# regras/NTT-based-polynomial-multiplier-FPGA

Hardware: AMD Instinct MI355X
Metric: polymults/sec (n=4096, 32-bit q) at 1/2/4/8 MI355X; % HBM roofline (higher is better)
Workload: dtype u32

## Files before the change

ntt-based-polynomial-multiplier-fpga_amd/csrc/arith_select.hpp:

```cpp
#pragma once
#include <stdint.h>

#ifndef NTTMUL_SPLIT16
#define NTTMUL_SPLIT16 4
#endif
#ifndef NTTMUL_C5_SQ
#define NTTMUL_C5_SQ 1
#endif

namespace nttmul {

constexpr int row_logs(int logn) {
  return logn <= 12 ? logn : (logn == 16 && NTTMUL_SPLIT16 == 5 ? 11 : 12);
}
constexpr int groups_g(int logs) { return (logs + 3) / 4; }
constexpr int groups_s(int logs, int g) {
  return logs / groups_g(logs) + (g < logs % groups_g(logs) ? 1 : 0);
}
constexpr bool p_signed_fw_entry(int logn, uint32_t idx) {
  if (idx < 2) return false;
  int st = 0;
  while ((2u << st) <= idx) st++;
  const int logs = row_logs(logn), local = st - (logn - logs);
  if (local < 0) return false;
  int g = 0, st0 = 0;
  while (st0 + groups_s(logs, g) <= local) st0 += groups_s(logs, g++);
  return local - st0 >= 1 && (idx & 1);
}

constexpr bool p3_fold_ok(uint64_t q) {
  if (q >= (1ull << 31) || q < 3) return false;
  const unsigned __int128 s1 = (unsigned __int128)4 * (q - 1) * (q - 1);
  const unsigned __int128 c32 = ((unsigned __int128)1 << 32) % q;
  const unsigned __int128 fold = (s1 >> 32) * c32 + 0xFFFFFFFFu;
  return fold + s1 < ((unsigned __int128)1 << 64);
}

enum class A32Kind { Plantard, Wide };

constexpr A32Kind a32_kind(uint64_t q) {
  return q >= (1ull << 31) ? A32Kind::Wide : A32Kind::Plantard;
}

}
```

ntt-based-polynomial-multiplier-fpga_amd/csrc/kernels.hip:

```cpp
#if defined(NTTMUL_HOOK_ROWS_LD) || defined(NTTMUL_HOOK_ROWS_ST) || defined(NTTMUL_HOOK_ROWS_INPUT) || \
    defined(NTTMUL_HOOK_ROWS_OUTPUT) || defined(NTTMUL_HOOK_XCHG) || defined(NTTMUL_HOOK_COLS_LD) || \
    defined(NTTMUL_HOOK_COLS_ST) || defined(NTTMUL_HOOK_TW) || defined(NTTMUL_HOOK_PRIO0)
#error "NTTMUL_HOOK_* are tools/kbench instrumentation points (wrong-result pricing builds), not library switches"
#endif
#include "kernels_dev.hpp"

namespace nttmul {

template <class T> struct Type { using type = T; };
template <class Tag> using type_of = typename Tag::type;

template <class F>
static hipError_t with_arith(const LaunchTables &T, F f) {
  if (T.word_bits == 32) {
    switch (a32_kind(T.q)) {
      case A32Kind::Wide: return f(Type<Arith32W>{});
      case A32Kind::Plantard: return f(Type<Arith32P>{});
    }
  }
  return f(Type<Arith64>{});
}

template <class F>
static hipError_t with_io(int io_bits, F f) {
  return io_bits == 64 ? f(Type<uint64_t>{}) : f(Type<uint32_t>{});
}

template <class A, class IO, int L1, int LOGS = 12>
static hipError_t multipass_l1(const LaunchTables &T, const void *a, const void *b, void *c,
                               size_t batch, void **scr, const Emit &E) {
  using W = typename A::word;
  const KParams<A> P = product_params<A>(T);
  const size_t cblocks = ((batch << LOGS) + 255) / 256;
  const auto name = [](const char *kernel) {
    return [kernel] {
      return std::string(kernel) + "<" + AName<A>::v + "," + word_name<IO>() + "," +
             std::to_string(L1) + ">";
    };
  };
  hipError_t e = emit(E, name("k_cols_fwd"), k_cols_fwd<A, IO, L1>, cblocks, 256, P, (const IO *)a,
                      (const IO *)b, (W *)scr[0], (W *)scr[1], batch, LOGS);
  if (e != hipSuccess) return e;
  e = launch_rows<A, W, W, LOGS, L1>(T, scr[0], scr[1], scr[2], batch << L1, E);
  if (e != hipSuccess) return e;
  return emit(E, name("k_cols_inv"), k_cols_inv<A, IO, L1>, cblocks, 256, P, (const W *)scr[2],
              (IO *)c, batch, LOGS);
}

template <class A, class IO>
static hipError_t multipass_sq(const LaunchTables &T, const void *a, const void *b, void *c,
                               size_t batch, void **scr, const Emit &E) {
  using W = typename A::word;
  const KParams<A> P = product_params<A>(T);
  const size_t groups = batch * 16;
  const auto name = [](const char *dir) {
    return [dir] {
      return std::string("k_cols8<") + AName<A>::v + "," + word_name<IO>() + "," + dir + ">";
    };
  };
  hipError_t e = emit(E, name("fwd"), k_cols8<A, IO, W, 0>, groups, 256, P, (const IO *)a,
                      (const IO *)b, (W *)scr[0], (W *)scr[1], groups);
  if (e != hipSuccess) return e;
  e = launch_rows<A, W, W, 8, 8>(T, scr[0], scr[1], scr[2], batch << 8, E);
  if (e != hipSuccess) return e;
  return emit(E, name("inv"), k_cols8<A, W, IO, 1>, groups, 256, P, (const W *)scr[2], nullptr,
              (IO *)c, nullptr, groups);
}

template <class A, class IO>
static hipError_t product(const LaunchTables &T, const void *a, const void *b, void *c,
                          size_t batch, void **scr, const Emit &E) {
  if constexpr (std::is_same<A, Arith32P>::value) {
    if (T.logn == 12 && p3_fold_ok(T.q))
      return launch_rows<Arith32P3, IO, IO, 12, 0>(T, a, b, c, batch, E);
  }
  if (T.logn <= 12)
    return with_logn(T.logn, [&](auto logs) {
      return launch_rows<A, IO, IO, decltype(logs)::value, 0>(T, a, b, c, batch, E);
    });
  if constexpr (sizeof(typename A::word) == 8 && NTTMUL_C5_SQ) {
    if (T.logn == 16) return multipass_sq<A, IO>(T, a, b, c, batch, scr, E);
  }
  switch (T.logn) {
    case 13: return multipass_l1<A, IO, 1>(T, a, b, c, batch, scr, E);
    case 14: return multipass_l1<A, IO, 2>(T, a, b, c, batch, scr, E);
// ... 182 lines not shown
```

ntt-based-polynomial-multiplier-fpga_amd/csrc/kernels_dev.hpp:

```cpp
#pragma once
#include <hip/hip_runtime.h>
#include <stdint.h>

#include <cstdlib>
#include <string>
#include <type_traits>

#include "launch.hpp"
#include "modarith.hpp"

#if defined(NTTMUL_HOOK_ROWS_LD) || defined(NTTMUL_HOOK_ROWS_ST)
#define NTTMUL_ROWS_HOOKED 1
#else
#define NTTMUL_ROWS_HOOKED 0
#endif
#ifndef NTTMUL_HOOK_ROWS_LD
#define NTTMUL_HOOK_ROWS_LD(base, u, N, b0) (base)
#endif
#ifndef NTTMUL_HOOK_ROWS_ST
#define NTTMUL_HOOK_ROWS_ST(base, u, N, b0) (base)
#endif
#ifndef NTTMUL_HOOK_ROWS_INPUT
#define NTTMUL_HOOK_ROWS_INPUT(x, y, u, j) do { } while (0)
#endif
#ifndef NTTMUL_HOOK_ROWS_OUTPUT
#define NTTMUL_HOOK_ROWS_OUTPUT(x, c, base, live) do { } while (0)
#endif
#ifndef NTTMUL_HOOK_PRIO0
#define NTTMUL_HOOK_PRIO0(u) __builtin_amdgcn_s_setprio(3)
#endif
#ifndef NTTMUL_HOOK_TW
#define NTTMUL_HOOK_TW(tw, idx, dir) ((tw)[idx])
#endif
#ifndef NTTMUL_HOOK_XCHG
#define NTTMUL_HOOK_XCHG() do { } while (0)
#endif
#if defined(NTTMUL_HOOK_COLS_LD) || defined(NTTMUL_HOOK_COLS_ST)
#define NTTMUL_COLS_HOOKED 1
#else
#define NTTMUL_COLS_HOOKED 0
#endif
#ifndef NTTMUL_HOOK_COLS_LD
#define NTTMUL_HOOK_COLS_LD(base, p, sh, col, dir) (base)
#endif
#ifndef NTTMUL_HOOK_COLS_ST
#define NTTMUL_HOOK_COLS_ST(base, p, sh, col) (base)
#endif

namespace nttmul {

template <class A>
struct KParams {
  A ar;
  const TwPair<typename A::word> *fw;
  const TwPair<typename A::word> *iw;
  typename A::word f, fs;
  typename A::word wf, wfs;
};

template <class A> struct AName;
template <class T> constexpr const char *word_name() { return sizeof(T) == 8 ? "u64" : "u32"; }

template <int LOGS>
struct Groups {
  static constexpr int N = 1 << LOGS;
  static constexpr int G = (LOGS + 3) / 4;
  static constexpr int S(int g) { return LOGS / G + (g < LOGS % G ? 1 : 0); }
  static constexpr int ST0(int g) {
    int s = 0;
    for (int i = 0; i < g; i++) s += S(i);
    return s;
  }
  static constexpr int NS(int g) { return 16 >> S(g); }
  static constexpr int LR(int g) { return LOGS - ST0(g) - S(g); }
  static constexpr int LNS(int g) { return 4 - S(g); }
  static constexpr int off(int g, int k) {
    int ns = NS(g), lr = LR(g), s = S(g);
    int m = k / ns, sidx = k % ns;
    if (lr >= LNS(g)) return sidx + (m << lr);
    return ((sidx >> lr) << (lr + s)) + (sidx & ((1 << lr) - 1)) + (m << lr);
  }
  __device__ static __forceinline__ int base(int g, int j) {
    int lr = LR(g), s = S(g), lns = LNS(g);
    if (lr >= lns) {
      int set0 = j << lns;
      return ((set0 >> lr) << (lr + s)) + (set0 & ((1 << lr) - 1));
    }
    return j << 4;
  }
  __device__ static __forceinline__ int blk(int g, int j, int k) {
    int lr = LR(g), lns = LNS(g);
    int sidx = k % NS(g);
    if (g == 0) return 0;
    if (lr >= lns) return (j << lns) >> lr;
    return (j << (lns - lr)) + (sidx >> lr);
  }
  static constexpr int reg_of(int g, int o) {
    for (int k = 0; k < 16; k++)
      if (off(g, k) == o) return k;
    return -1;
  }
  static constexpr bool kPad0 = LOGS >= 10 && G > 2;
  static constexpr bool kPad2 = LOGS == 10 || LOGS == 9;
  static constexpr int PS(int x) {
    return kPad2 ? (LOGS == 10 ? (x == 0 ? 6 : 4) : (x == 0 ? 5 : 4))
                 : (x == 0 && kPad0 ? LOGS - 4 : 4);
  }
  static constexpr int PT(int x) {
    return kPad2 ? (LOGS == 10 ? (x == 0 ? 3 : 1) : (x == 0 ? 0 : 1))
                 : (x == 0 && kPad0 ? LOGS - 8 : 0);
  }
  static constexpr int PS2(int x) { return kPad2 ? (LOGS == 10 ? 8 : (x == 0 ? 7 : 8)) : 31; }
  template <int X>
  static constexpr int padx(int e) { return e + ((e >> PS(X)) << PT(X)) + (e >> PS2(X)); }
  static constexpr int pad(int e) { return padx<1>(e); }
  static constexpr int NP = (padx<0>(N - 1) > padx<1>(N - 1) ? padx<0>(N - 1) : padx<1>(N - 1)) + 1 >
                                    N + N / 16
                                ? (padx<0>(N - 1) > padx<1>(N - 1) ? padx<0>(N - 1) : padx<1>(N - 1)) + 1
                                : N + N / 16;
};

template <int LOGS>
constexpr bool groups_agree() {
  for (int g = 0; g < Groups<LOGS>::G; g++)
    if (Groups<LOGS>::S(g) != groups_s(LOGS, g)) return false;
  return Groups<LOGS>::G == groups_g(LOGS);
}
static_assert(groups_agree<8>() && groups_agree<9>() && groups_agree<10>() && groups_agree<11>() &&
                  groups_agree<12>(),
              "arith_select.hpp's group helpers (planner twiddle forms) must match Groups<>");

template <class W, class T>
__device__ __forceinline__ W to_word(T v) { return (W)v; }

template <class A>
struct IsPlantard : std::false_type {};
template <>
struct IsPlantard<Arith32P> : std::true_type {};
template <>
struct IsPlantard<Arith32P3> : std::true_type {};
template <> struct AName<Arith32P> { static constexpr const char *v = "Arith32P"; };
template <> struct AName<Arith32P3> { static constexpr const char *v = "Arith32P3"; };
template <> struct AName<Arith32W> { static constexpr const char *v = "Arith32W"; };
template <> struct AName<Arith64> { static constexpr const char *v = "Arith64"; };

template <bool NT, class T>
__device__ __forceinline__ T ld_stream(const T *p) {
  if constexpr (NT) return __builtin_nontemporal_load(p);
  return *p;
}
template <bool NT, class T>
__device__ __forceinline__ void st_stream(T *p, T v) {
  if constexpr (NT)
    __builtin_nontemporal_store(v, p);
  else
    *p = v;
}

constexpr int kAuxNt = 2;
template <class T>
__device__ __forceinline__ auto span_rsrc(const T *p, size_t words) {
  return __builtin_amdgcn_make_buffer_rsrc((void *)p, 0, (int)(words * sizeof(T)), 0x00020000);
}
template <int AUX, class R>
__device__ __forceinline__ uint32_t buf_ld32(R r, int byte_off, int soff = 0) {
  return __builtin_amdgcn_raw_buffer_load_b32(r, byte_off, soff, AUX);
}
template <int AUX, class R>
__device__ __forceinline__ void buf_st32(R r, int byte_off, uint32_t v, int soff = 0) {
  __builtin_amdgcn_raw_buffer_store_b32(v, r, byte_off, soff, AUX);
}
template <int AUX, class R>
__device__ __forceinline__ uint64_t buf_ld64(R r, int byte_off, int soff) {
  typedef unsigned int u2 __attribute__((ext_vector_type(2)));
  const u2 v = __builtin_amdgcn_raw_buffer_load_b64(r, byte_off, soff, AUX);
  return ((uint64_t)v.y << 32) | v.x;
}
template <int AUX, class R>
__device__ __forceinline__ void buf_st64(R r, int byte_off, uint64_t v, int soff) {
  typedef unsigned int u2 __attribute__((ext_vector_type(2)));
  const u2 w = {(unsigned)v, (unsigned)(v >> 32)};
  __builtin_amdgcn_raw_buffer_store_b64(w, r, byte_off, soff, AUX);
}

template <class A, int LOGS, int g, int NPOLY, int SKIP>
__device__ __forceinline__ void fwd_stage(const A &ar, typename A::word (&x)[16],
                                          typename A::word (&y)[16],
                                          const TwPair<typename A::word> *__restrict__ tw, int j,
                                          int row, int l1, TwPair<typename A::word> (&zw)[16],
                                          int l) {
  using Gr = Groups<LOGS>;
  constexpr int S = Gr::S(g), st0 = Gr::ST0(g), ns = Gr::NS(g);
  const int dist = 8 >> l;
  const int st = st0 + l;
  const int tbase = (1 << (l1 + st)) + (row << st);
#pragma unroll
  for (int k = 0; k < 16; k++) {
    if (k & dist) continue;
    const int m = k / ns;
    const int idx = tbase + (Gr::blk(g, j, k) << l) + (m >> (S - l));
    const TwPair<typename A::word> t = NTTMUL_HOOK_TW(tw, idx, 0);
    if (l == S - SKIP - 1) zw[k] = t;
    const bool xc = g == 0 && l == 0 && l1 == 0;
    if constexpr (IsPlantard<A>::value) {
      const bool xn = l > 0 && (k & (2 * dist)) != 0;
      const bool yn = l < S - SKIP - 1 || (SKIP > 0 && g + 1 == Gr::G);
#define NTTMUL_CT_P(XC_, XN_, YN_)                                         \
  do {                                                                     \
    ar.template ct<XC_, XN_, YN_>(x[k], x[k + dist], t.w, t.ws);            \
    if (NPOLY == 2) ar.template ct<XC_, XN_, YN_>(y[k], y[k + dist], t.w, t.ws); \
  } while (0)
      if (xc) {
        if (yn) NTTMUL_CT_P(true, false, true); else NTTMUL_CT_P(true, false, false);
// ... 3 lines not shown
        if (yn) NTTMUL_CT_P(false, false, true); else NTTMUL_CT_P(false, false, false);
      }
#undef NTTMUL_CT_P
      continue;
    }
    if (xc) {
      ar.template ct<true>(x[k], x[k + dist], t.w, t.ws);
      if (NPOLY == 2) ar.template ct<true>(y[k], y[k + dist], t.w, t.ws);
    } else {
      ar.ct(x[k], x[k + dist], t.w, t.ws);
      if (NPOLY == 2) ar.ct(y[k], y[k + dist], t.w, t.ws);
    }
  }
}

template <class A, int LOGS, int g, int NPOLY = 2, int SKIP = 0, int L = 0>
__device__ __forceinline__ void fwd_group(const A &ar, typename A::word (&x)[16],
                                          typename A::word (&y)[16],
                                          const TwPair<typename A::word> *__restrict__ tw, int j,
                                          int row, int l1,
                                          TwPair<typename A::word> (&zw)[16]) {
  using Gr = Groups<LOGS>;
  constexpr int S = Gr::S(g);
  if constexpr (sizeof(typename A::word) == 8) {
    if constexpr (L < S - SKIP) {
      fwd_stage<A, LOGS, g, NPOLY, SKIP>(ar, x, y, tw, j, row, l1, zw, L);
      fwd_group<A, LOGS, g, NPOLY, SKIP, L + 1>(ar, x, y, tw, j, row, l1, zw);
    }
  } else {
#pragma unroll
    for (int l = 0; l < S - SKIP; l++)
      fwd_stage<A, LOGS, g, NPOLY, SKIP>(ar, x, y, tw, j, row, l1, zw, l);
  }
}

template <class A, int LOGS, int g, bool SCALE, int SKIP>
__device__ __forceinline__ void inv_stage(const KParams<A> &P, typename A::word (&x)[16],
                                          const TwPair<typename A::word> *__restrict__ tw, int j,
                                          int row, int l1, int l) {
  using Gr = Groups<LOGS>;
  constexpr int S = Gr::S(g), st0 = Gr::ST0(g), ns = Gr::NS(g);
  const int dist = 8 >> l;
  const int st = st0 + l;
  const int tbase = (1 << (l1 + st)) + (row << st);
#pragma unroll
  for (int k = 0; k < 16; k++) {
    if (k & dist) continue;
    if (SCALE && st == 0) {
      P.ar.gs_scaled(x[k], x[k + dist], P.f, P.fs, P.wf, P.wfs);
    } else {
      const int m = k / ns;
      const int idx = tbase + (Gr::blk(g, j, k) << l) + (m >> (S - l));
      const TwPair<typename A::word> t = NTTMUL_HOOK_TW(tw, idx, 1);
      P.ar.gs(x[k], x[k + dist], t.w, t.ws);
    }
  }
}

template <class A, int LOGS, int g, bool SCALE, int SKIP = 0, int L = Groups<LOGS>::S(g) - 1 - SKIP>
__device__ __forceinline__ void inv_group(const KParams<A> &P, typename A::word (&x)[16],
                                          const TwPair<typename A::word> *__restrict__ tw, int j,
                                          int row, int l1) {
  if constexpr (sizeof(typename A::word) == 8) {
    if constexpr (L >= 0) {
      inv_stage<A, LOGS, g, SCALE, SKIP>(P, x, tw, j, row, l1, L);
      inv_group<A, LOGS, g, SCALE, SKIP, L - 1>(P, x, tw, j, row, l1);
    }
  } else {
#pragma unroll
    for (int l = L; l >= 0; l--) inv_stage<A, LOGS, g, SCALE, SKIP>(P, x, tw, j, row, l1, l);
  }
}

template <int SYNC>
__device__ __forceinline__ void xsync() {
  if constexpr (SYNC == 0) {
    __syncthreads();
  } else {
    __builtin_amdgcn_fence(__ATOMIC_ACQ_REL, "wavefront");
    __builtin_amdgcn_wave_barrier();
  }
}


template <int LOGS, int gfrom, int gto, int NREG, class W, int SYNC = 0, int ES = 1>
__device__ __forceinline__ void exchange(W (&x)[16], W (&y)[16], W *lds, int j) {
  using Gr = Groups<LOGS>;
  NTTMUL_HOOK_XCHG();
  constexpr int X = gfrom < gto ? gfrom : gto;
  const int bw = Gr::template padx<X>(Gr::base(gfrom, j)) * ES;
  const int br = Gr::template padx<X>(Gr::base(gto, j)) * ES;
#pragma unroll
  for (int k = 0; k < 16; k++) lds[bw + Gr::template padx<X>(Gr::off(gfrom, k)) * ES] = x[k];
  xsync<SYNC>();
#pragma unroll
  for (int k = 0; k < 16; k++) x[k] = lds[br + Gr::template padx<X>(Gr::off(gto, k)) * ES];
  xsync<SYNC>();
  if constexpr (NREG == 2) {
#pragma unroll
    for (int k = 0; k < 16; k++) lds[bw + Gr::template padx<X>(Gr::off(gfrom, k)) * ES] = y[k];
    xsync<SYNC>();
#pragma unroll
    for (int k = 0; k < 16; k++) y[k] = lds[br + Gr::template padx<X>(Gr::off(gto, k)) * ES];
    xsync<SYNC>();
  }
}

template <class A, int LOGS, int g, int NPOLY = 2, int SKIP = 0, int SYNC = 0, int ES = 1>
__device__ __forceinline__ void fwd_all(const A &ar, typename A::word (&x)[16],
                                        typename A::word (&y)[16], typename A::word *lds,
                                        const TwPair<typename A::word> *__restrict__ tw, int j,
                                        int row, int l1, TwPair<typename A::word> (&zw)[16]) {
  using Gr = Groups<LOGS>;
  constexpr bool last = g + 1 == Gr::G;
  fwd_group<A, LOGS, g, NPOLY, last ? SKIP : 0>(ar, x, y, tw, j, row, l1, zw);
  if constexpr (!last) {
    exchange<LOGS, g, g + 1, NPOLY, typename A::word, SYNC, ES>(x, y, lds, j);
    fwd_all<A, LOGS, g + 1, NPOLY, SKIP, SYNC, ES>(ar, x, y, lds, tw, j, row, l1, zw);
  }
}

template <class A, int LOGS, int g, bool SCALE, int SKIP = 0, int SYNC = 0, int NPOLY = 1,
          int ES = 1>
__device__ __forceinline__ void inv_all(const KParams<A> &P, typename A::word (&x)[16],
                                        typename A::word (&y)[16], typename A::word *lds,
                                        const TwPair<typename A::word> *__restrict__ tw, int j,
                                        int row, int l1) {
  using Gr = Groups<LOGS>;
  inv_group<A, LOGS, g, SCALE, g + 1 == Gr::G ? SKIP : 0>(P, x, tw, j, row, l1);
  if constexpr (NPOLY == 2) inv_group<A, LOGS, g, SCALE, g + 1 == Gr::G ? SKIP : 0>(P, y, tw, j, row, l1);
  if constexpr (g > 0) {
    exchange<LOGS, g, g - 1, NPOLY, typename A::word, SYNC, ES>(x, y, lds, j);
    inv_all<A, LOGS, g - 1, SCALE, SKIP, SYNC, NPOLY, ES>(P, x, y, lds, tw, j, row, l1);
  }
}

template <class A, int LOGS, int D, int K0 = 0>
__device__ __forceinline__ void base_mult_rec(const A &ar, typename A::word (&x)[16],
                                          const typename A::word (&y)[16],
                                          const TwPair<typename A::word> (&zw)[16]) {
  using Gr = Groups<LOGS>;
  constexpr int g = Gr::G - 1, B = 1 << D;
  static_assert(D > 0 && Gr::S(g) > D, "base blocks of 2^D > 1 coefficients in the last group");
  if constexpr (K0 < 16) {
    constexpr int o0 = Gr::off(g, K0);
    if constexpr ((o0 & (B - 1)) == 0) {
      int r[B];
#pragma unroll
      for (int i = 0; i < B; i++) r[i] = Gr::reg_of(g, o0 + i);
      constexpr bool neg = (o0 >> D) & 1;
      constexpr int kz = Gr::reg_of(g, o0 & ~B);
      const TwPair<typename A::word> z = zw[kz];
      constexpr int dl = 8 >> (Gr::S(g) - D - 1);
      constexpr bool zc = IsPlantard<A>::value && Gr::S(g) - D - 1 > 0 && (kz & (2 * dl));
      typename A::word a[B], b[B];
#pragma unroll
      for (int i = 0; i < B; i++) a[i] = x[r[i]], b[i] = y[r[i]];
      ar.template basemul<B, neg, zc>(a, b, z.w, z.ws);
#pragma unroll
      for (int i = 0; i < B; i++) x[r[i]] = a[i];
    }
    base_mult_rec<A, LOGS, D, K0 + 1>(ar, x, y, zw);
  }
}

template <class A, int LOGS, int D>
__device__ __forceinline__ void base_mult(const A &ar, typename A::word (&x)[16],
                                          const typename A::word (&y)[16],
                                          const TwPair<typename A::word> (&zw)[16]) {
  using Gr = Groups<LOGS>;
  constexpr int g = Gr::G - 1, B = 1 << D;
  static_assert(D == 0 || Gr::S(g) > D, "last register group too short for the base blocks");
  if constexpr (D == 0) {
#pragma unroll
    for (int k = 0; k < 16; k++) x[k] = ar.mont(x[k], y[k]);
  } else if constexpr (std::is_same<A, Arith32P3>::value) {
    base_mult_rec<A, LOGS, D>(ar, x, y, zw);
  } else {
#pragma unroll
    for (int k0 = 0; k0 < 16; k0++) {
      const int o0 = Gr::off(g, k0);
      if (o0 & (B - 1)) continue;
      int r[B];
#pragma unroll
      for (int i = 0; i < B; i++) r[i] = Gr::reg_of(g, o0 + i);
      const bool neg = (o0 >> D) & 1;
      const int kz = Gr::reg_of(g, o0 & ~B);
      const TwPair<typename A::word> z = zw[kz];
      constexpr int dl = 8 >> (Gr::S(g) - D - 1);
      const bool zc = IsPlantard<A>::value && Gr::S(g) - D - 1 > 0 && (kz & (2 * dl));
      typename A::word a[B], b[B];
#pragma unroll
      for (int i = 0; i < B; i++) a[i] = x[r[i]], b[i] = y[r[i]];
      if (zc) {
        if (neg)
          ar.template basemul<B, true, true>(a, b, z.w, z.ws);
        else
          ar.template basemul<B, false, true>(a, b, z.w, z.ws);
      } else if (neg)
        ar.template basemul<B, true>(a, b, z.w, z.ws);
      else
        ar.template basemul<B, false>(a, b, z.w, z.ws);
#pragma unroll
      for (int i = 0; i < B; i++) x[r[i]] = a[i];
    }
  }
}

__host__ __device__ constexpr int rows_threads(int logs) { return logs == 10 ? 64 : 256; }
__host__ __device__ constexpr bool c8_tile(int logs, int l1) { return logs == 8 && l1 == 8; }


#ifdef NTTMUL_CLOCK_STAMPS
constexpr unsigned kClkSlots = 1u << 16;
__device__ unsigned long long g_clk[kClkSlots * 4];
hipError_t read_clock_stamps(void *dst, size_t blocks) {
  return hipMemcpyFromSymbol(dst, HIP_SYMBOL(g_clk),
                             (blocks < kClkSlots ? blocks : kClkSlots) * 4 * sizeof(unsigned long long));
}
__device__ __forceinline__ void clk_stamp(int k) {
  if (threadIdx.x == 0) {
    unsigned long long t, r;
    __builtin_amdgcn_sched_barrier(0);
    asm volatile("s_memtime %0\n\ts_memrealtime %1\n\ts_waitcnt lgkmcnt(0)" : "=s"(t), "=s"(r)::"memory");
    __builtin_amdgcn_sched_barrier(0);
    unsigned long long *p = g_clk + (blockIdx.x % kClkSlots) * 4 + 2 * k;
    p[0] = t;
    p[1] = r;
  }
}
#define CLK_STAMP(k) clk_stamp(k)
#else
#define CLK_STAMP(k) do { } while (0)
#endif

template <class A, class TIn, class TOut, int LOGS, int L1, bool PRIO = false>
__global__ __launch_bounds__(rows_threads(LOGS)) void k_rows(
    KParams<A> P, const TIn *__restrict__ a, const TIn *__restrict__ b, TOut *__restrict__ c,
    size_t units) {
  using W = typename A::word;
  using Gr = Groups<LOGS>;
  constexpr int N = Gr::N, TP = N / 16, PB = rows_threads(LOGS) / TP, G = Gr::G, NP = Gr::NP;
  constexpr bool kNT = L1 == 0;
  __shared__ W lds[PB][NP];

  const int pb = threadIdx.x / TP, j = threadIdx.x % TP;
  const size_t u = (size_t)blockIdx.x * PB + pb;
  const bool live = u < units;
  const int row = L1 ? (int)(u & ((1u << L1) - 1)) : 0;
  constexpr bool kTile = c8_tile(LOGS, L1);
  constexpr int kRS = kTile ? 256 : 1;
  const size_t base_g = kTile ? ((u >> 8) << 16) + ((u & 255) << 4) + Gr::base(0, j)
                              : u * N + Gr::base(0, j);
  const size_t base_l = live ? base_g : (size_t)Gr::base(0, j);
  const size_t base_r = NTTMUL_HOOK_ROWS_LD(base_l, u, N, Gr::base(0, j));

  constexpr bool kRowBuf = kTile && !NTTMUL_ROWS_HOOKED && sizeof(W) == 8 && sizeof(TIn) == 8 &&
                           sizeof(TOut) == 8;
  const size_t rpoly = (((size_t)blockIdx.x * PB) >> 8) << 16;
  const int rlane = (int)(((u & 255) << 4) + Gr::base(0, j));
  CLK_STAMP(0);
  if constexpr (PRIO) NTTMUL_HOOK_PRIO0(u);
  W x[16], y[16];
  constexpr bool kCpol = PB == 1 && L1 == 0 && sizeof(W) == 4 && sizeof(TIn) == 4 &&
                         sizeof(TOut) == 4;
  if constexpr (kCpol) {
    const size_t ub = live ? (size_t)blockIdx.x : 0;
    const auto ra = span_rsrc(a + ub * N, N), rb = span_rsrc(b + ub * N, N);
#pragma unroll
    for (int k = 0; k < 16; k++) {
      const int vo = Gr::base(0, j) * 4, so = Gr::off(0, k) * 4;
      x[k] = (W)buf_ld32<kAuxNt>(ra, vo, so);
      y[k] = (W)buf_ld32<kAuxNt>(rb, vo, so);
    }
  } else if constexpr (kRowBuf) {
    const auto ra = span_rsrc(a + rpoly, 65536), rb = span_rsrc(b + rpoly, 65536);
#pragma unroll
    for (int k = 0; k < 16; k++) {
      const int so = Gr::off(0, k) * kRS * 8;
      x[k] = (W)buf_ld64<0>(ra, rlane * 8, so);
      y[k] = (W)buf_ld64<0>(rb, rlane * 8, so);
    }
  } else {
#pragma unroll
    for (int k = 0; k < 16; k++) {
      x[k] = to_word<W>(ld_stream<kNT>(a + base_r + Gr::off(0, k) * kRS));
      y[k] = to_word<W>(ld_stream<kNT>(b + base_r + Gr::off(0, k) * kRS));
    }
  }
  NTTMUL_HOOK_ROWS_INPUT(x, y, u, j);
  W *lx = lds[pb];
  constexpr int D = A::kBaseD;
  TwPair<W> zw[16];
  fwd_all<A, LOGS, 0, 2, D>(P.ar, x, y, lx, P.fw, j, row, L1, zw);
  if constexpr (PRIO) __builtin_amdgcn_s_setprio(1);
  base_mult<A, LOGS, D>(P.ar, x, y, zw);
  if constexpr (PRIO) __builtin_amdgcn_s_setprio(0);
  inv_all<A, LOGS, G - 1, L1 == 0, D>(P, x, y, lx, P.iw, j, row, L1);
  NTTMUL_HOOK_ROWS_OUTPUT(x, c, base_g, live);
  if constexpr (kCpol) {
    if (live) {
      const auto rc = span_rsrc(c + (size_t)blockIdx.x * N, N);
#pragma unroll
      for (int k = 0; k < 16; k++) {
        W v = x[k];
        if (!A::kInvCanonical) v = P.ar.canon_inv(v);
        buf_st32<kAuxNt>(rc, Gr::base(0, j) * 4, (uint32_t)v, Gr::off(0, k) * 4);
      }
    }
    CLK_STAMP(1);
    return;
  }
  if constexpr (kRowBuf) {
    const auto rc = span_rsrc(c + rpoly, 65536);
#pragma unroll
    for (int k = 0; k < 16; k++) buf_st64<0>(rc, rlane * 8, (uint64_t)x[k], Gr::off(0, k) * kRS * 8);
    CLK_STAMP(1);
    return;
  }
  if (live) {
    const size_t base_w = NTTMUL_HOOK_ROWS_ST(base_g, u, N, Gr::base(0, j));
#pragma unroll
    for (int k = 0; k < 16; k++) {
      W v = x[k];
      if (L1 == 0 && !A::kInvCanonical) v = P.ar.canon_inv(v);
      st_stream<kNT>(c + base_w + Gr::off(0, k) * kRS, (TOut)v);
    }
  }
  CLK_STAMP(1);
}

constexpr int kServerPollSleep = 2;
template <int P_>
__device__ __forceinline__ int wl_elem(int t, int i) {
  return (t & ((1 << P_) - 1)) | ((t >> P_) << (P_ + 2)) | (i << P_);
}
__device__ __forceinline__ int wl_pad(int e) { return e + (e >> 5); }
template <int PF, int PT>
__device__ __forceinline__ void wl_exchange(uint32_t (&x)[4], uint32_t *lx, int t) {
#pragma unroll
  for (int i = 0; i < 4; i++) lx[wl_pad(wl_elem<PF>(t, i))] = x[i];
  xsync<1>();
#pragma unroll
  for (int i = 0; i < 4; i++) x[i] = lx[wl_pad(wl_elem<PT>(t, i))];
  xsync<1>();
}
struct WideTw {
  TwPair<uint32_t> f[9], z, i[8];
};
__device__ __forceinline__ WideTw wide_tw(const TwPair<uint32_t> *fu, const TwPair<uint32_t> *fs,
                                          const TwPair<uint32_t> *iw, int t) {
  WideTw w;
  const int k3 = 8 + ((t >> 4) << 1), k5 = 32 + ((t >> 2) << 1);
  w.f[0] = fu[1];
  w.f[1] = fu[2];
  w.f[2] = fs[3];
  w.f[3] = fu[4 + (t >> 4)];
  w.f[4] = fu[k3];
  w.f[5] = fs[k3 + 1];
  w.f[6] = fu[16 + (t >> 2)];
  w.f[7] = fu[k5];
  w.f[8] = fs[k5 + 1];
  w.z = fs[32 + (t >> 1)];
  w.i[0] = iw[k5];
  w.i[1] = iw[k5 + 1];
  w.i[2] = iw[16 + (t >> 2)];
  w.i[3] = iw[k3];
  w.i[4] = iw[k3 + 1];
  w.i[5] = iw[4 + (t >> 4)];
  w.i[6] = iw[2];
  w.i[7] = iw[3];
  return w;
}
__device__ __forceinline__ void wl_swap_64(uint32_t (&x)[4]) {
  auto s0 = __builtin_amdgcn_permlane16_swap(x[0], x[1], false, false);
  auto s1 = __builtin_amdgcn_permlane16_swap(x[2], x[3], false, false);
  x[0] = s0[0], x[1] = s0[1], x[2] = s1[0], x[3] = s1[1];
  auto s2 = __builtin_amdgcn_permlane32_swap(x[0], x[2], false, false);
  auto s3 = __builtin_amdgcn_permlane32_swap(x[1], x[3], false, false);
  x[0] = s2[0], x[2] = s2[1], x[1] = s3[0], x[3] = s3[1];
}
// ... 245 lines not shown
      if (split) {
        fwd_all<A, LOGS, 0, 1, D, 1>(P.ar, x, y, lx, P.fw, j, 0, 0, zw);
#pragma unroll
        for (int k = 0; k < 16; k++)
          y[k] = (W)__builtin_amdgcn_ds_bpermute((lane + TP) << 2, (int)x[k]);
      } else {
        fwd_all<A, LOGS, 0, 2, D, 1>(P.ar, x, y, lx, P.fw, j, 0, 0, zw);
      }
      base_mult<A, LOGS, D>(P.ar, x, y, zw);
      inv_all<A, LOGS, G - 1, true, D, 1>(P, x, y, lx, P.iw, j, 0, 0);
#ifdef NTTMUL_CLOCK_STAMPS
      __builtin_amdgcn_sched_barrier(0);
      st[2] = __builtin_amdgcn_s_memrealtime();
      st[5] = __builtin_amdgcn_s_memtime();
#endif
      W *sc = (W *)stg[0];
      if (live) {
        const int base = pb * N + Gr::base(0, j);
#pragma unroll
        for (int k = 0; k < 16; k++) {
          W v = x[k];
          if (!A::kInvCanonical) v = P.ar.canon_inv(v);
          sc[base + Gr::off(0, k)] = v;
        }
      }
      xsync<1>();
      const auto rc = span_rsrc(box->c, KW);
      for (int i = lane; i < q4; i += 64) {
        const uint4 v = stg[0][i];
        __attribute__((ext_vector_type(4))) uint32_t w = {v.x, v.y, v.z, v.w};
        __builtin_amdgcn_raw_buffer_store_b128(w, rc, i * 16, 0, 17);
      }
    }
#ifdef NTTMUL_CLOCK_STAMPS
    if (wave == 0) {
      __builtin_amdgcn_fence(__ATOMIC_RELEASE, "");
      asm volatile("s_waitcnt vmcnt(0)" ::: "memory");
      st[3] = __builtin_amdgcn_s_memrealtime();
      if (threadIdx.x == 0)
        for (int k = 0; k < 6; k++) box->stamp[k] = st[k];
      __builtin_amdgcn_fence(__ATOMIC_RELEASE, "");
      asm volatile("s_waitcnt vmcnt(0)" ::: "memory");
      __hip_atomic_store(&box->done, go, __ATOMIC_RELAXED, __HIP_MEMORY_SCOPE_SYSTEM);
    }
#endif
    seen = go;
    last = now;
    if constexpr (NT > 64) __syncthreads(); else xsync<1>();
  }
}

template <class A, int L1, int DIR>
constexpr int xform_upg() { return L1 == 0 && sizeof(typename A::word) == 4 ? 2 : 1; }
template <class A, class TIn, class TOut, int LOGS, int L1, int DIR>
__global__ __launch_bounds__(256) void k_xform(KParams<A> P, const TIn *__restrict__ in,
                                               TOut *__restrict__ out, size_t units) {
  using W = typename A::word;
  using Gr = Groups<LOGS>;
  constexpr int N = Gr::N, TP = N / 16, PB = 256 / TP, G = Gr::G, NP = Gr::NP;
  constexpr int GIN = DIR == 0 ? 0 : G - 1, GOUT = DIR == 0 ? G - 1 : 0;
  constexpr int UPG = xform_upg<A, L1, DIR>();
  __shared__ W lds[PB][UPG][NP];
  const int pb = threadIdx.x / TP, j = threadIdx.x % TP;
  const size_t u = ((size_t)blockIdx.x * PB + pb) * UPG;
  const bool live = u < units, live2 = UPG == 2 && u + 1 < units;
  const int row = L1 ? (int)(u & ((1u << L1) - 1)) : 0;
  constexpr bool kTile = c8_tile(LOGS, L1);
  constexpr int kRS = kTile ? 256 : 1;
  static_assert(!kTile || UPG == 1, "one polynomial per thread group on the tiled layout");
  const auto tbase = [&](size_t v, int g) {
    return kTile ? ((v >> 8) << 16) + ((v & 255) << 4) + Gr::base(g, j) : v * N + Gr::base(g, j);
  };
  const size_t base_in = DIR == 0 ? tbase(live ? u : 0, GIN) : (live ? u : 0) * N + Gr::base(GIN, j);
  const size_t base_in2 = (live2 ? u + 1 : live ? u : 0) * N + Gr::base(GIN, j);
  constexpr int kRSI = DIR == 0 ? kRS : 1, kRSO = DIR == 1 ? kRS : 1;
  W x[16], y[16];
#pragma unroll
  for (int k = 0; k < 16; k++) {
    x[k] = to_word<W>(in[base_in + Gr::off(GIN, k) * kRSI]);
    if (UPG == 2) y[k] = to_word<W>(in[base_in2 + Gr::off(GIN, k)]);
  }
  TwPair<W> zw[16];
  if (DIR == 0)
    fwd_all<A, LOGS, 0, UPG>(P.ar, x, y, lds[pb][0], P.fw, j, row, L1, zw);
  else
    inv_all<A, LOGS, G - 1, L1 == 0, 0, 0, UPG>(P, x, y, lds[pb][0], P.iw, j, row, L1);
  if (live) {
    const size_t base_out = DIR == 1 ? tbase(u, GOUT) : u * N + Gr::base(GOUT, j);
#pragma unroll
    for (int k = 0; k < 16; k++) {
      W v = x[k];
      if (DIR == 0)
        v = P.ar.canon(v);
      else if (L1 == 0 && !A::kInvCanonical)
        v = P.ar.canon_inv(v);
      out[base_out + Gr::off(GOUT, k) * kRSO] = (TOut)v;
    }
  }
  if (live2) {
    const size_t base_out = (u + 1) * N + Gr::base(GOUT, j);
#pragma unroll
    for (int k = 0; k < 16; k++) {
      W v = y[k];
      if (DIR == 0)
        v = P.ar.canon(v);
      else if (!A::kInvCanonical)
        v = P.ar.canon_inv(v);
      out[base_out + Gr::off(GOUT, k)] = (TOut)v;
    }
  }
}

template <class A, class IO>
__global__ __launch_bounds__(256) void k_pointwise(KParams<A> P, const IO *__restrict__ a,
                                                   const IO *__restrict__ b, IO *__restrict__ c,
                                                   size_t total) {
  using W = typename A::word;
  const size_t i = (size_t)blockIdx.x * blockDim.x + threadIdx.x;
  if (i >= total) return;
  const W t = P.ar.mont((W)a[i], (W)b[i]);
  c[i] = (IO)P.ar.canon_inv(P.ar.mont(t, P.f));
}

template <class A, class TIn, int L1, int NPOLY = 2>
__global__ __launch_bounds__(256) void k_cols_fwd(KParams<A> P, const TIn *__restrict__ a,
                                                  const TIn *__restrict__ b,
                                                  typename A::word *__restrict__ ta,
                                                  typename A::word *__restrict__ tb, size_t batch,
                                                  int logs) {
  using W = typename A::word;
  constexpr int M = 1 << L1;
  const size_t ncol = (size_t)1 << logs;
  const size_t gid = (size_t)blockIdx.x * blockDim.x + threadIdx.x;
  if (gid >= batch * ncol) return;
  const size_t p = gid >> logs, col = gid & (ncol - 1);
  const size_t base = (p << (logs + L1)) + col;
  const size_t base_r = NTTMUL_HOOK_COLS_LD(base, p, logs + L1, col, 0);
  const size_t base_w = NTTMUL_HOOK_COLS_ST(base, p, logs + L1, col);
  W x[M], y[M];
#pragma clang loop unroll(full)
  for (int m = 0; m < M; m++) {
    x[m] = (W)ld_stream<true>(a + base_r + ((size_t)m << logs));
    y[m] = NPOLY == 2 ? (W)ld_stream<true>(b + base_r + ((size_t)m << logs)) : W(0);
  }
#pragma clang loop unroll(full)
  for (int st = 0; st < L1; st++) {
    const int dist = M >> (st + 1);
#pragma clang loop unroll(full)
    for (int m = 0; m < M; m++) {
      if (m & dist) continue;
      const TwPair<W> t = P.fw[(1 << st) + (m >> (L1 - st))];
      P.ar.ct(x[m], x[m + dist], t.w, t.ws);
      if (NPOLY == 2) P.ar.ct(y[m], y[m + dist], t.w, t.ws);
    }
  }
#pragma clang loop unroll(full)
  for (int m = 0; m < M; m++) {
    st_stream<true>(ta + base_w + ((size_t)m << logs), x[m]);
    if (NPOLY == 2) st_stream<true>(tb + base_w + ((size_t)m << logs), y[m]);
  }
}

template <class A, class TOut, int L1>
__global__ __launch_bounds__(256) void k_cols_inv(KParams<A> P,
                                                  const typename A::word *__restrict__ tc,
                                                  TOut *__restrict__ c, size_t batch, int logs) {
  using W = typename A::word;
  constexpr int M = 1 << L1;
  const size_t ncol = (size_t)1 << logs;
// ... 254 lines not shown
```

Measured before the change: 68.31 million.

## Scope LDS exchange barriers to wave level when data stays inside one wave

Adds compile-time analysis of whether each LDS exchange between NTT groups keeps data within a single 64-lane wave. Such exchanges now use wave-scope sync instead of workgroup barriers, with one extra workgroup barrier placed where a wave-local exchange is followed by a cross-wave one. The trailing barrier after the last exchange is dropped in tail positions. The aim is to cut workgroup barrier stalls in the row NTT kernels at n=4096. The risk is LDS race bugs if the hazard analysis is wrong.

```diff
diff --git a/ntt-based-polynomial-multiplier-fpga_amd/csrc/arith_select.hpp b/ntt-based-polynomial-multiplier-fpga_amd/csrc/arith_select.hpp
--- a/ntt-based-polynomial-multiplier-fpga_amd/csrc/arith_select.hpp
+++ b/ntt-based-polynomial-multiplier-fpga_amd/csrc/arith_select.hpp
@@ -17,6 +17,46 @@
 constexpr int groups_s(int logs, int g) {
   return logs / groups_g(logs) + (g < logs % groups_g(logs) ? 1 : 0);
 }
+constexpr int groups_st0(int logs, int g) {
+  int s = 0;
+  for (int i = 0; i < g; i++) s += groups_s(logs, i);
+  return s;
+}
+constexpr int groups_lr(int logs, int g) { return logs - groups_st0(logs, g) - groups_s(logs, g); }
+constexpr int groups_off(int logs, int g, int k) {
+  const int s = groups_s(logs, g), ns = 16 >> s, lr = groups_lr(logs, g);
+  const int m = k / ns, sidx = k % ns;
+  if (lr >= 4 - s) return sidx + (m << lr);
+  return ((sidx >> lr) << (lr + s)) + (sidx & ((1 << lr) - 1)) + (m << lr);
+}
+constexpr int groups_base(int logs, int g, int j) {
+  const int s = groups_s(logs, g), lns = 4 - s, lr = groups_lr(logs, g);
+  if (lr < lns) return j << 4;
+  const int set0 = j << lns;
+  return ((set0 >> lr) << (lr + s)) + (set0 & ((1 << lr) - 1));
+}
+constexpr bool exchange_wave_local(int logs, int x, int ts = 1) {
+  const int tp = (1 << logs) / 16;
+  if (x < 0 || x + 1 >= groups_g(logs) || logs > 12) return false;
+  if (tp * ts <= 64) return true;
+  int wave[4096] = {}, o0[16] = {}, o1[16] = {};
+  for (int k = 0; k < 16; k++) o0[k] = groups_off(logs, x, k), o1[k] = groups_off(logs, x + 1, k);
+  for (int j = 0; j < tp; j++) {
+    const int b = groups_base(logs, x, j);
+    for (int k = 0; k < 16; k++) wave[b + o0[k]] = j * ts / 64;
+  }
+  for (int j = 0; j < tp; j++) {
+    const int b = groups_base(logs, x + 1, j), w = j * ts / 64;
+    for (int k = 0; k < 16; k++)
+      if (wave[b + o1[k]] != w) return false;
+  }
+  return true;
+}
+constexpr bool exchange_lead_barrier(int logs, int x, int prev, int ts = 1) {
+  if (prev < 0 || (1 << logs) / 16 * ts <= 64 || !exchange_wave_local(logs, prev, ts)) return false;
+  return !(prev == x);
+}
+
 constexpr bool p_signed_fw_entry(int logn, uint32_t idx) {
   if (idx < 2) return false;
   int st = 0;
diff --git a/ntt-based-polynomial-multiplier-fpga_amd/csrc/kernels.hip b/ntt-based-polynomial-multiplier-fpga_amd/csrc/kernels.hip
--- a/ntt-based-polynomial-multiplier-fpga_amd/csrc/kernels.hip
+++ b/ntt-based-polynomial-multiplier-fpga_amd/csrc/kernels.hip
@@ -1,6 +1,7 @@
 #if defined(NTTMUL_HOOK_ROWS_LD) || defined(NTTMUL_HOOK_ROWS_ST) || defined(NTTMUL_HOOK_ROWS_INPUT) || \
     defined(NTTMUL_HOOK_ROWS_OUTPUT) || defined(NTTMUL_HOOK_XCHG) || defined(NTTMUL_HOOK_COLS_LD) || \
-    defined(NTTMUL_HOOK_COLS_ST) || defined(NTTMUL_HOOK_TW) || defined(NTTMUL_HOOK_PRIO0)
+    defined(NTTMUL_HOOK_COLS_ST) || defined(NTTMUL_HOOK_TW) || defined(NTTMUL_HOOK_PRIO0) || \
+    defined(NTTMUL_HOOK_XCHG_SYNC)
 #error "NTTMUL_HOOK_* are tools/kbench instrumentation points (wrong-result pricing builds), not library switches"
 #endif
 #include "kernels_dev.hpp"
diff --git a/ntt-based-polynomial-multiplier-fpga_amd/csrc/kernels_dev.hpp b/ntt-based-polynomial-multiplier-fpga_amd/csrc/kernels_dev.hpp
--- a/ntt-based-polynomial-multiplier-fpga_amd/csrc/kernels_dev.hpp
+++ b/ntt-based-polynomial-multiplier-fpga_amd/csrc/kernels_dev.hpp
@@ -34,6 +34,9 @@
 #endif
 #ifndef NTTMUL_HOOK_XCHG
 #define NTTMUL_HOOK_XCHG() do { } while (0)
+#endif
+#ifndef NTTMUL_HOOK_XCHG_SYNC
+#define NTTMUL_HOOK_XCHG_SYNC(sync) (sync)
 #endif
 #if defined(NTTMUL_HOOK_COLS_LD) || defined(NTTMUL_HOOK_COLS_ST)
 #define NTTMUL_COLS_HOOKED 1
@@ -80,7 +83,7 @@
     if (lr >= LNS(g)) return sidx + (m << lr);
     return ((sidx >> lr) << (lr + s)) + (sidx & ((1 << lr) - 1)) + (m << lr);
   }
-  __device__ static __forceinline__ int base(int g, int j) {
+  __host__ __device__ static constexpr __forceinline__ int base(int g, int j) {
     int lr = LR(g), s = S(g), lns = LNS(g);
     if (lr >= lns) {
       int set0 = j << lns;
@@ -118,17 +121,53 @@
                                     N + N / 16
                                 ? (padx<0>(N - 1) > padx<1>(N - 1) ? padx<0>(N - 1) : padx<1>(N - 1)) + 1
                                 : N + N / 16;
+  static constexpr bool wave_local(int X, int TS = 1) {
+    if (X < 0 || X + 1 >= G) return false;
+    if (N / 16 * TS <= 64) return true;
+    int holder[N] = {}, o0[16] = {}, o1[16] = {};
+    for (int k = 0; k < 16; k++) o0[k] = off(X, k), o1[k] = off(X + 1, k);
+    for (int j = 0; j < N / 16; j++) {
+      const int b = base(X, j);
+      for (int k = 0; k < 16; k++) holder[b + o0[k]] = j * TS / 64;
+    }
+    for (int j = 0; j < N / 16; j++) {
+      const int b = base(X + 1, j), w = j * TS / 64;
+      for (int k = 0; k < 16; k++)
+        if (holder[b + o1[k]] != w) return false;
+    }
+    return true;
+  }
 };
 
 template <int LOGS>
 constexpr bool groups_agree() {
   for (int g = 0; g < Groups<LOGS>::G; g++)
     if (Groups<LOGS>::S(g) != groups_s(LOGS, g)) return false;
+  for (int ts = 1; ts <= 16; ts *= 16)
+    for (int x = -1; x < Groups<LOGS>::G; x++)
+      if (Groups<LOGS>::wave_local(x, ts) != exchange_wave_local(LOGS, x, ts)) return false;
   return Groups<LOGS>::G == groups_g(LOGS);
 }
-static_assert(groups_agree<8>() && groups_agree<9>() && groups_agree<10>() && groups_agree<11>() &&
-                  groups_agree<12>(),
-              "arith_select.hpp's group helpers (planner twiddle forms) must match Groups<>");
+#define NTTMUL_GROUPS_AGREE(L) \
+  static_assert(groups_agree<L>(), \
+                "arith_select.hpp's group helpers (planner twiddle forms, exchange scopes) must match Groups<>")
+NTTMUL_GROUPS_AGREE(8);
+NTTMUL_GROUPS_AGREE(9);
+NTTMUL_GROUPS_AGREE(10);
+NTTMUL_GROUPS_AGREE(11);
+NTTMUL_GROUPS_AGREE(12);
+#undef NTTMUL_GROUPS_AGREE
+static_assert(exchange_wave_local(8, 0) && exchange_wave_local(9, 0) && exchange_wave_local(9, 1) &&
+                  exchange_wave_local(10, 0) && exchange_wave_local(10, 1),
+              "rows of at most 64 threads exchange inside their wave");
+static_assert(!exchange_wave_local(11, 0) && exchange_wave_local(11, 1) &&
+                  !exchange_wave_local(12, 0) && exchange_wave_local(12, 1),
+              "n = 2048 / 4096: exchange 0 crosses waves, exchange 1 stays inside one");
+static_assert(exchange_lead_barrier(12, 0, 1) && exchange_lead_barrier(11, 0, 1) &&
+                  !exchange_lead_barrier(12, 1, 1) && !exchange_lead_barrier(12, 1, 0) &&
+                  !exchange_lead_barrier(12, 0, -1) && !exchange_lead_barrier(9, 0, 1),
+              "the one extra workgroup barrier: before 1 -> 0 after the wave-scope 2 -> 1");
+static_assert(!exchange_wave_local(8, 0, 16), "k_cols8's exchange crosses waves");
 
 template <class W, class T>
 __device__ __forceinline__ W to_word(T v) { return (W)v; }
@@ -298,31 +337,36 @@
   }
 }
 
-
-template <int LOGS, int gfrom, int gto, int NREG, class W, int SYNC = 0, int ES = 1>
+template <int LOGS, int gfrom, int gto, int NREG, class W, int SYNC_ = 0, int ES = 1, int PREV = -1,
+          bool TAIL = false>
 __device__ __forceinline__ void exchange(W (&x)[16], W (&y)[16], W *lds, int j) {
   using Gr = Groups<LOGS>;
   NTTMUL_HOOK_XCHG();
   constexpr int X = gfrom < gto ? gfrom : gto;
+  constexpr int SYNC = NTTMUL_HOOK_XCHG_SYNC(SYNC_);
+  constexpr bool kAuto = SYNC == 0;
+  constexpr int SC = SYNC == 1 || (kAuto && Gr::wave_local(X, ES)) ? 1 : 0;
   const int bw = Gr::template padx<X>(Gr::base(gfrom, j)) * ES;
   const int br = Gr::template padx<X>(Gr::base(gto, j)) * ES;
+  if constexpr (kAuto && exchange_lead_barrier(LOGS, X, PREV, ES)) xsync<0>();
 #pragma unroll
   for (int k = 0; k < 16; k++) lds[bw + Gr::template padx<X>(Gr::off(gfrom, k)) * ES] = x[k];
-  xsync<SYNC>();
+  xsync<SC>();
 #pragma unroll
   for (int k = 0; k < 16; k++) x[k] = lds[br + Gr::template padx<X>(Gr::off(gto, k)) * ES];
-  xsync<SYNC>();
   if constexpr (NREG == 2) {
+    xsync<SC>();
 #pragma unroll
     for (int k = 0; k < 16; k++) lds[bw + Gr::template padx<X>(Gr::off(gfrom, k)) * ES] = y[k];
-    xsync<SYNC>();
+    xsync<SC>();
 #pragma unroll
     for (int k = 0; k < 16; k++) y[k] = lds[br + Gr::template padx<X>(Gr::off(gto, k)) * ES];
-    xsync<SYNC>();
-  }
-}
-
-template <class A, int LOGS, int g, int NPOLY = 2, int SKIP = 0, int SYNC = 0, int ES = 1>
+  }
+  if constexpr (!(kAuto && TAIL)) xsync<SC>();
+}
+
+template <class A, int LOGS, int g, int NPOLY = 2, int SKIP = 0, int SYNC = 0, int ES = 1,
+          int PREV = -1, bool TAIL = false>
 __device__ __forceinline__ void fwd_all(const A &ar, typename A::word (&x)[16],
                                         typename A::word (&y)[16], typename A::word *lds,
                                         const TwPair<typename A::word> *__restrict__ tw, int j,
@@ -331,13 +375,14 @@
   constexpr bool last = g + 1 == Gr::G;
   fwd_group<A, LOGS, g, NPOLY, last ? SKIP : 0>(ar, x, y, tw, j, row, l1, zw);
   if constexpr (!last) {
-    exchange<LOGS, g, g + 1, NPOLY, typename A::word, SYNC, ES>(x, y, lds, j);
-    fwd_all<A, LOGS, g + 1, NPOLY, SKIP, SYNC, ES>(ar, x, y, lds, tw, j, row, l1, zw);
+    exchange<LOGS, g, g + 1, NPOLY, typename A::word, SYNC, ES, PREV, TAIL && g + 2 == Gr::G>(
+        x, y, lds, j);
+    fwd_all<A, LOGS, g + 1, NPOLY, SKIP, SYNC, ES, g, TAIL>(ar, x, y, lds, tw, j, row, l1, zw);
   }
 }
 
 template <class A, int LOGS, int g, bool SCALE, int SKIP = 0, int SYNC = 0, int NPOLY = 1,
-          int ES = 1>
+          int ES = 1, int PREV = -1, bool TAIL = false>
 __device__ __forceinline__ void inv_all(const KParams<A> &P, typename A::word (&x)[16],
                                         typename A::word (&y)[16], typename A::word *lds,
                                         const TwPair<typename A::word> *__restrict__ tw, int j,
@@ -346,8 +391,8 @@
   inv_group<A, LOGS, g, SCALE, g + 1 == Gr::G ? SKIP : 0>(P, x, tw, j, row, l1);
   if constexpr (NPOLY == 2) inv_group<A, LOGS, g, SCALE, g + 1 == Gr::G ? SKIP : 0>(P, y, tw, j, row, l1);
   if constexpr (g > 0) {
-    exchange<LOGS, g, g - 1, NPOLY, typename A::word, SYNC, ES>(x, y, lds, j);
-    inv_all<A, LOGS, g - 1, SCALE, SKIP, SYNC, NPOLY, ES>(P, x, y, lds, tw, j, row, l1);
+    exchange<LOGS, g, g - 1, NPOLY, typename A::word, SYNC, ES, PREV, TAIL && g == 1>(x, y, lds, j);
+    inv_all<A, LOGS, g - 1, SCALE, SKIP, SYNC, NPOLY, ES, g - 1, TAIL>(P, x, y, lds, tw, j, row, l1);
   }
 }
 
@@ -508,11 +553,12 @@
   W *lx = lds[pb];
   constexpr int D = A::kBaseD;
   TwPair<W> zw[16];
-  fwd_all<A, LOGS, 0, 2, D>(P.ar, x, y, lx, P.fw, j, row, L1, zw);
+  constexpr int kXS = rows_threads(LOGS) == 64 ? 2 : 0;
+  fwd_all<A, LOGS, 0, 2, D, kXS>(P.ar, x, y, lx, P.fw, j, row, L1, zw);
   if constexpr (PRIO) __builtin_amdgcn_s_setprio(1);
   base_mult<A, LOGS, D>(P.ar, x, y, zw);
   if constexpr (PRIO) __builtin_amdgcn_s_setprio(0);
-  inv_all<A, LOGS, G - 1, L1 == 0, D>(P, x, y, lx, P.iw, j, row, L1);
+  inv_all<A, LOGS, G - 1, L1 == 0, D, kXS, 1, 1, G - 2, true>(P, x, y, lx, P.iw, j, row, L1);
   NTTMUL_HOOK_ROWS_OUTPUT(x, c, base_g, live);
   if constexpr (kCpol) {
     if (live) {
@@ -924,9 +970,9 @@
   }
   TwPair<W> zw[16];
   if (DIR == 0)
-    fwd_all<A, LOGS, 0, UPG>(P.ar, x, y, lds[pb][0], P.fw, j, row, L1, zw);
+    fwd_all<A, LOGS, 0, UPG, 0, 0, 1, -1, true>(P.ar, x, y, lds[pb][0], P.fw, j, row, L1, zw);
   else
-    inv_all<A, LOGS, G - 1, L1 == 0, 0, 0, UPG>(P, x, y, lds[pb][0], P.iw, j, row, L1);
+    inv_all<A, LOGS, G - 1, L1 == 0, 0, 0, UPG, 1, -1, true>(P, x, y, lds[pb][0], P.iw, j, row, L1);
   if (live) {
     const size_t base_out = DIR == 1 ? tbase(u, GOUT) : u * N + Gr::base(GOUT, j);
 #pragma unroll
```

Result: no change. 68.29 million (-0.0%).
